# anonymous-author-918/deq-mpc-corl

Hardware: AMD Instinct MI355X
Metric: QP solves/sec at (B,T=20,nx=13,nu=4) (higher is better)
Workload: dtype f32

## Files before the change

deq-mpc-corl_amd/_lib.py:

```python
from __future__ import annotations

import ctypes as C
import os

_HERE = os.path.dirname(os.path.abspath(__file__))
LIB_PATH = os.environ.get("MI_ALQP_LIB") or os.path.join(_HERE, "csrc", "libmi_alqp.so")

ABI_VERSION = 10


class AlqpDims(C.Structure):
    _fields_ = [("B", C.c_int), ("T", C.c_int), ("nx", C.c_int), ("nu", C.c_int)]


class AlqpParams(C.Structure):
    _fields_ = [("al_iter", C.c_int), ("max_newton", C.c_int), ("n_ls", C.c_int),
                ("flags", C.c_int), ("rho_scale", C.c_double), ("variant", C.c_int),
                ("skip_flag", C.c_void_p), ("exit_tol", C.c_double), ("newton_counts", C.c_void_p),
                ("exit_scratch", C.c_void_p), ("quad_stagger", C.c_int)]


class AlqpTrace(C.Structure):
    _fields_ = [("g", C.c_void_p), ("d", C.c_void_p), ("phi", C.c_void_p),
                ("phi_prev", C.c_void_p), ("k", C.c_void_p), ("accept", C.c_void_p)]


class AlqpObstacles(C.Structure):
    _fields_ = [("pos", C.c_void_p), ("radius", C.c_double), ("nobs", C.c_int), ("state_estimator", C.c_int)]


class AlqpIpmParams(C.Structure):
    _fields_ = [("flags", C.c_int), ("max_iter", C.c_int), ("iter0", C.c_int), ("kkt_eps", C.c_double),
                ("variant", C.c_int)]


class AlqpRigidParams(C.Structure):
    _fields_ = [("mass", C.c_double), ("J", C.c_double * 9), ("Jinv", C.c_double * 9), ("g", C.c_double * 3),
                ("motor_dist", C.c_double), ("kf", C.c_double), ("bf", C.c_double), ("km", C.c_double),
                ("act_scale", C.c_double), ("u_hover", C.c_double), ("pend_L", C.c_double), ("ss", C.c_double * 12),
                ("bf_force", C.c_double)]


IPM_VARIANTS = {"auto": 0, "generic_lds": 1, "generic_ws": 2, "resident": 3}


ALQP_IPM_INIT, ALQP_IPM_RESID, ALQP_IPM_STEP, ALQP_IPM_LOOP, ALQP_IPM_FINAL = 1, 2, 4, 8, 16
ALQP_INIT_MERIT = 1
ALQP_DUAL_UPDATE = 2
ALQP_SAVE_FACTOR = 4
ALQP_WS_PRIMED = 8
ALQP_EXIT_IN_KERNEL = 16
ALQP_E_COOP = -4
# ... 19 lines not shown
                                   C.c_long, C.c_long, _P, _P, _P, _P, _P]),
    "alqp_merit": (C.c_int, [C.POINTER(AlqpDims), C.c_int, _P, _P, _P, _P, _P, _P, _P, _P, _P,
                             C.c_long, C.c_long, _P, _P, _P]),
    "alqp_linesearch_pick": (C.c_int, [C.POINTER(AlqpDims), C.c_int, _P, _P, _P, _P, _P, _P, _P]),
    "alqp_dual_update": (C.c_int, [C.POINTER(AlqpDims), _P, _P, _P, _P, _P, C.c_long, C.c_long, _P, _P,
                                   C.c_double, _P]),
    "alqp_backward": (C.c_int, [C.POINTER(AlqpDims), _P, _P, _P, _P, _P, _P, _P, _P]),
    "alqp_backward_ws": (C.c_int, [C.POINTER(AlqpDims), _P, C.c_size_t, _P, _P, _P, _P, _P, _P, _P]),
    "alqp_newton_step_obs": (C.c_int, [C.POINTER(AlqpDims), _P, _P, _P, _P, _P, _P, _P, _P, _P, _P,
                                       C.c_long, C.c_long, C.POINTER(AlqpObstacles), _P, _P, _P, _P, _P]),
    "alqp_merit_obs": (C.c_int, [C.POINTER(AlqpDims), C.c_int, _P, _P, _P, _P, _P, _P, _P, _P, _P,
                                 C.c_long, C.c_long, C.POINTER(AlqpObstacles), _P, _P, _P]),
    "alqp_dual_update_obs": (C.c_int, [C.POINTER(AlqpDims), _P, _P, _P, _P, _P, C.c_long, C.c_long,
                                       C.POINTER(AlqpObstacles), _P, _P, C.c_double, _P]),
    "alqp_newton_step_ws": (C.c_int, [C.POINTER(AlqpDims), _P, _P, _P, _P, _P, _P, _P, _P, _P, _P,
                                      C.c_long, C.c_long, _P, C.c_size_t, _P, _P, _P, _P]),
    "alqp_newton_step_ws_obs": (C.c_int, [C.POINTER(AlqpDims), _P, _P, _P, _P, _P, _P, _P, _P, _P, _P,
                                          C.c_long, C.c_long, C.POINTER(AlqpObstacles), _P, C.c_size_t, _P, _P, _P, _P]),
    "alqp_merit_pick": (C.c_int, [C.POINTER(AlqpDims), C.c_int, _P, _P, _P, _P, _P, _P, _P, _P, _P,
                                  C.c_long, C.c_long, C.POINTER(AlqpObstacles), _P, _P, _P, _P, _P, _P, _P]),
    "alqp_ipm_solve": (C.c_int, [C.POINTER(AlqpDims), C.POINTER(AlqpIpmParams), _P, _P, _P, _P, _P, _P, _P,
                                 C.c_long, C.c_long, C.c_long, C.c_long, C.c_long, C.c_long, _P, C.c_size_t, _P,
                                 _P, _P, _P, _P, _P, _P, _P, _P, _P, _P]),
    "alqp_ipm_backward": (C.c_int, [C.POINTER(AlqpDims), _P, _P, C.c_long, C.c_long, C.c_long, C.c_long, _P, _P, _P,
                                    _P, C.c_size_t, _P, _P, _P, _P, C.c_int, _P]),
}
_PLAIN = {
    "alqp_abi_version": (C.c_int, []),
    "alqp_supported": (C.c_int, [C.POINTER(AlqpDims), C.c_int]),
    "alqp_supported_variant": (C.c_int, [C.POINTER(AlqpDims), C.c_int, C.c_int]),
    "alqp_lds_bytes": (C.c_size_t, [C.POINTER(AlqpDims), C.c_int]),
    "alqp_qps_per_wave": (C.c_int, [C.POINTER(AlqpDims), C.c_int]),
    "alqp_workspace_bytes": (C.c_size_t, [C.POINTER(AlqpDims), C.c_int]),
    "alqp_exit_test": (C.c_int, [C.c_void_p, C.c_void_p, C.c_int, C.c_double, C.c_void_p]),
    "alqp_workspace_bytes_nonlin": (C.c_size_t, [C.POINTER(AlqpDims), C.c_int]),
    "alqp_ipm_workspace_bytes": (C.c_size_t, [C.POINTER(AlqpDims), C.c_int]),
}

EXPORTED_SYMBOLS = sorted([f"{n}_{s}" for n in _SIGS for s in ("f32", "f64")] + list(_PLAIN))

_lib = None


def load():
    global _lib
    if _lib is not None:
        return _lib
    if not os.path.exists(LIB_PATH):
        raise RuntimeError(
            f"mi_alqp: HIP extension not built ({LIB_PATH} missing). Run "
            "`python -c 'import __graft_entry__ as g; g.build()'` - there is no CPU fallback.")
    lib = C.CDLL(LIB_PATH)
    for name, (res, args) in _SIGS.items():
        for sfx in ("f32", "f64"):
            fn = getattr(lib, f"{name}_{sfx}")
            fn.restype = res
            fn.argtypes = args
    for name, (res, args) in _PLAIN.items():
        fn = getattr(lib, name)
        fn.restype = res
        fn.argtypes = args
    if lib.alqp_abi_version() != ABI_VERSION:
        raise RuntimeError("mi_alqp: libmi_alqp.so ABI version mismatch - rebuild the extension")
    _lib = lib
    return lib

# ... 5 lines not shown
```

deq-mpc-corl_amd/backend.py:

```python
from __future__ import annotations

import ctypes as C

import os

import torch

from . import _lib


def _dt(t):
    if t.dtype == torch.float32:
        return "f32"
    if t.dtype == torch.float64:
        return "f64"
    raise TypeError(f"mi_alqp: unsupported dtype {t.dtype}")


def _ptr(t, name, dtype=None, allow_none=False):
    if t is None:
        if allow_none:
            return None
        raise ValueError(f"mi_alqp: {name} is required")
    if not t.is_cuda:
# ... 15 lines not shown


class HipBackend:

    name = "hip"
    supports_exit_in_kernel = True
    default_variant = "auto"
    QUAD_MIN_BATCH = 4096

    def __init__(self):
        self.lib = _lib.load()
        self._ws = {}
        if os.environ.get("ALQP_QUAD_STAGGER") is not None:
            self.set_quad_stagger(int(os.environ["ALQP_QUAD_STAGGER"]))

    quad_stagger = -1

    def set_quad_stagger(self, mode):
        prev, self.quad_stagger = self.quad_stagger, (-1 if int(mode) < 0 else int(mode))
        return prev

    def workspace_bytes(self, B, T, nx, nu, dtype):
        d = _lib.AlqpDims(B, T, nx, nu)
        return int(self.lib.alqp_workspace_bytes(C.byref(d), int(dtype == torch.float64)))

    def _workspace(self, dims, like):
        need = self.workspace_bytes(*dims, like.dtype)
        key = (like.device, like.dtype)
        ws = self._ws.get(key)
        if ws is None or ws.numel() * ws.element_size() < need:
            ws = torch.empty(need // like.element_size() + 16, dtype=like.dtype, device=like.device)
            self._ws[key] = ws
        return ws, need

    def supported(self, B, T, nx, nu, dtype):
        d = _lib.AlqpDims(B, T, nx, nu)
        return bool(self.lib.alqp_supported(C.byref(d), int(dtype == torch.float64)))

    def lds_bytes(self, B, T, nx, nu, dtype):
        d = _lib.AlqpDims(B, T, nx, nu)
        return int(self.lib.alqp_lds_bytes(C.byref(d), int(dtype == torch.float64)))

    def qps_per_wave(self, B, T, nx, nu, dtype):
        d = _lib.AlqpDims(B, T, nx, nu)
        return int(self.lib.alqp_qps_per_wave(C.byref(d), int(dtype == torch.float64)))

    def solve_lin(self, dims, Qd, q, F, c, x0, ulo, uhi, sb_u, st_u, z, lam, rho, phi,
                  rnorm2=None, info=None, status=None, factor=None, al_iter=2, max_newton=4,
                  n_ls=20, flags=_lib.ALQP_INIT_MERIT | _lib.ALQP_DUAL_UPDATE, rho_scale=10.0,
                  trace=None, variant=None, workspace=None, skip=None, newton_counts=None, exit_tol=1e-3):
        B, T, nx, nu = dims
        dt = z.dtype
        sfx = _dt(z)
        d = _lib.AlqpDims(B, T, nx, nu)
        if variant is None:
            variant = self.default_variant
        vnum = {"auto": 0, "team": 1, "quad": 2}[variant]
        if vnum == 0:
            if self.QUAD_MIN_BATCH != 4096:
                qmin = self.QUAD_MIN_BATCH
            elif 2 * (nx + nu) + nx + 1 > 32:
                qmin = 4097
            else:
                qmin = 4608 if dt == torch.float64 else 4096
            vnum = 1 if ((flags & _lib.ALQP_SAVE_FACTOR) or B < qmin) else 2
            if vnum == 1 and not (flags & _lib.ALQP_SAVE_FACTOR) and not self.lib.alqp_supported_variant(C.byref(d), int(dt == torch.float64), 1):
                vnum = 2
        ws, ws_bytes = (None, 0)
        if vnum == 2:
            if workspace is not None:
                ws, ws_bytes = workspace, self.workspace_bytes(*dims, z.dtype)
                if ws.numel() * ws.element_size() < ws_bytes:
                    raise ValueError("mi_alqp: workspace too small")
            else:
                ws, ws_bytes = self._workspace(dims, z)
        self.last_variant = "quad" if vnum == 2 else "team"
        skp = _ptr(skip, "skip", torch.float64, True)
        p = _lib.AlqpParams(al_iter, max_newton, n_ls, flags | _DEBUG_FLAGS, rho_scale, vnum, skp.value if skp is not None else None)
        p.quad_stagger = {-1: 0, 0: -1}.get(self.quad_stagger, self.quad_stagger)
        if newton_counts is not None:
            self._exit_in_kernel(p, B, z.device, newton_counts, exit_tol)
        tr = None
        if trace is not None:
            tr = _lib.AlqpTrace(*[
                (trace[k].data_ptr() if trace.get(k) is not None else None)
                for k in ("g", "d", "phi", "phi_prev", "k", "accept")])
        fn = getattr(self.lib, "alqp_solve_lin_" + sfx)
        rc = fn(C.byref(d), C.byref(p), _ptr(Qd, "Qd", dt), _ptr(q, "q", dt), _ptr(F, "F", dt),
                _ptr(c, "c", dt), _ptr(x0, "x0", dt), _ptr(ulo, "u_lower", dt), _ptr(uhi, "u_upper", dt),
                sb_u, st_u, _ptr(z, "z", dt), _ptr(lam, "lam", dt), _ptr(rho, "rho", dt),
                _ptr(phi, "phi", dt), _ptr(rnorm2, "rnorm2", dt, True),
                _ptr(info, "info", torch.int32, True), _ptr(status, "status", torch.uint8, True),
                _ptr(factor, "factor", dt, True), C.byref(tr) if tr is not None else None,
                _ptr(ws, "workspace", dt, True), ws_bytes, _stream())
        if rc == _lib.ALQP_E_COOP and newton_counts is not None:
            return False
        _lib.check(rc, "alqp_solve_lin_" + sfx)
        return True

    def _exit_in_kernel(self, p, B, device, newton_counts, exit_tol):
        key = ("exit", device)
        scr = self._ws.get(key)
        if scr is None or scr.numel() < 2 * B + 2:
            scr = torch.zeros(2 * B + 2, dtype=torch.float64, device=device)
            self._ws[key] = scr
        scr.zero_()
        p.flags |= _lib.ALQP_EXIT_IN_KERNEL
        p.exit_tol = float(exit_tol)
        p.newton_counts = _ptr(newton_counts, "newton_counts", torch.int32).value
        p.exit_scratch = scr.data_ptr()

    def solve_nonlin(self, dims, dyn_id, dyn_h, Qd, q, x0, ulo, uhi, sb_u, st_u, z, lam, rho, phi, rnorm2=None,
# ... 337 lines not shown
```

deq-mpc-corl_amd/csrc/alqp_kernels.hip:

```cpp
#include <hip/hip_runtime.h>

#include "alqp_team.hpp"
#include "alqp_quad.hpp"
#include "mi_alqp.h"
#include "alqp_dims.hpp"

#ifndef ALQP_PART
#define ALQP_PART 0
#endif
#define ALQP_BUILD_MAIN (ALQP_PART == 0 || ALQP_PART == 1)
#define ALQP_BUILD_QUAD (ALQP_PART == 0 || ALQP_PART == 2 || ALQP_PART == 3)
#define ALQP_QUAD_F32 (ALQP_PART == 0 || ALQP_PART == 2)
#define ALQP_QUAD_F64 (ALQP_PART == 0 || ALQP_PART == 3)

#include <hip/hip_cooperative_groups.h>

namespace alqp {

template <typename real>
struct SolveArgs {
    int B, T;
    int al_iter, max_newton, n_ls, flags;
    real rho_scale;
    const real *Qd, *q, *F, *c, *x0, *ulo, *uhi;
    long sb_u, st_u;
    real *z, *lam, *rho, *phi, *rnorm2;
    int *info;
    unsigned char *status;
    real *factor;
    const double *skip;
    real dyn_h;
    int stagger;
    double exit_tol;
    int *newton_counts;
    double *exit_scratch;
};

__device__ inline double grid_sum_ordered(double block_val, double *scratch, int &phase) {
    double *p = scratch + 1 + (size_t)(phase & 1) * gridDim.x;
    unsigned *cnt = reinterpret_cast<unsigned *>(scratch);
    double *timed_out = scratch + 1 + 2 * (size_t)gridDim.x;
    if (threadIdx.x == 0) {
        __hip_atomic_store(p + blockIdx.x, block_val, __ATOMIC_RELAXED, __HIP_MEMORY_SCOPE_AGENT);
        __hip_atomic_fetch_add(cnt, 1u, __ATOMIC_RELEASE, __HIP_MEMORY_SCOPE_AGENT);
        const unsigned target = (unsigned)(phase + 1) * gridDim.x;
        if (__hip_atomic_load(timed_out, __ATOMIC_RELAXED, __HIP_MEMORY_SCOPE_AGENT) == 0.0) {
            const unsigned long long t0 = __builtin_amdgcn_s_memrealtime();
            bool late = false;
            while (__hip_atomic_load(cnt, __ATOMIC_RELAXED, __HIP_MEMORY_SCOPE_AGENT) < target) {
                __builtin_amdgcn_s_sleep(2);
                if (__builtin_amdgcn_s_memrealtime() - t0 > 100000000ull ||
                    __hip_atomic_load(timed_out, __ATOMIC_RELAXED, __HIP_MEMORY_SCOPE_AGENT) != 0.0) { late = true; break; }
            }
            if (late) __hip_atomic_store(timed_out, 1.0, __ATOMIC_RELAXED, __HIP_MEMORY_SCOPE_AGENT);
            else (void)__hip_atomic_load(cnt, __ATOMIC_ACQUIRE, __HIP_MEMORY_SCOPE_AGENT);
        }
    }
    __builtin_amdgcn_s_barrier();
    if (__hip_atomic_load(timed_out, __ATOMIC_RELAXED, __HIP_MEMORY_SCOPE_AGENT) != 0.0) {
        ++phase;
        return __builtin_nan("");
    }
    double s = 0;
    for (unsigned i = threadIdx.x; i < gridDim.x; i += 64) s += __hip_atomic_load(p + i, __ATOMIC_RELAXED, __HIP_MEMORY_SCOPE_AGENT);
#pragma unroll
    for (int off = 32; off; off >>= 1) s += __shfl_xor(s, off, 64);
    ++phase;
    return s;
// ... 190 lines not shown
    }

    const real rn2 = tm.rplus2();
    int bad = 0;
    for (int e = li; e < T * N; e += G) {
        real v = tm.zs[e];
        bad |= !(v - v == real(0));
    }
    bad = team_or<G>(bad);
#ifdef ALQP_PHASE_TIMING
    tm.stamp(7);
    if (lane == 0)
        for (int i = 0; i < 8; ++i) atomicAdd(&g_team_cycles[i], tm.tacc[i]);
#endif
    if (active) {
        for (int e = li; e < T * N; e += G) gz[e] = tm.zs[e];
        if ((a.flags & ALQP_SAVE_FACTOR) && a.factor) {
            real *gf = a.factor + (size_t)b * T * C::XT;
            for (int e = li; e < T * C::XT; e += G) gf[e] = tm.Xp[e];
        }
        if (li == 0) {
            a.rho[b] = tm.rho;
            a.phi[b] = phi_prev;
            if (a.rnorm2) a.rnorm2[b] = rn2;
            if (a.info && tm.info && a.info[b] == 0) a.info[b] = tm.info;
            if (a.status) a.status[b] = bad ? 0 : 1;
        }
    }
}

#endif

#if ALQP_BUILD_QUAD
#ifndef ALQP_FUSE_LS
#define ALQP_FUSE_LS 1
#endif
#ifdef ALQP_PHASE_TIMING
__device__ unsigned long long g_phase_cycles[10];
#define QSTAMP(b) qd.stamp(b)
#else
#define QSTAMP(b)
#endif
template <typename real, int NX, int NU, bool TRACE, class Dyn = NoDyn>
__global__ __launch_bounds__(64) __attribute__((amdgpu_waves_per_eu(1, 1))) void k_solve_lin_quad(SolveArgs<real> a, TraceArgs<real> tr, real *ws) {
    using C = QCfg<real, NX, NU>;
    constexpr bool NL = Dyn::ID != 0;
#ifndef ALQP_FUSE_LS_F64
#define ALQP_FUSE_LS_F64 1
#endif
    constexpr bool FUSE_LS = ALQP_FUSE_LS && (sizeof(real) == 4 || ALQP_FUSE_LS_F64) && !NL;
    constexpr int N = C::N;
    if (a.skip && *a.skip != 0.0) return;
    const int lane = threadIdx.x, qi = lane >> 2;
    const int b_raw = blockIdx.x * 16 + qi;
    const bool active = b_raw < a.B;
    {
        int stag = a.stagger;
        const int mode = (a.flags >> 20) & 0xf;
        if ((a.flags >> 24) & 0xff) stag = (a.flags >> 24) & 0xff;
        if (stag > 0) {
            const unsigned hw = __builtin_amdgcn_s_getreg(4 | (0 << 6) | (31 << 11));
            int simd = (hw >> 4) & 3;
            if (mode == 1) simd = simd * 16 + ((hw >> 8) & 0xf);
            if (mode == 2) simd &= 1;
            if (mode == 3) simd = blockIdx.x & 1;
            if (mode == 4) simd = (simd & 1) ^ (blockIdx.x & 1);
            if (mode == 5) simd = (hw >> 8) & 3;
            for (int i = 0; i < simd * stag; ++i) __builtin_amdgcn_s_sleep(16);
        }
    }
#ifdef ALQP_ALIAS_ALL
    const int b = (active ? b_raw : a.B - 1) % ALQP_ALIAS_ALL;
#else
    const int b = active ? b_raw : a.B - 1;
#endif
    const int T = a.T, M = C::M(T);

    Quad<real, NX, NU> qd;
    __shared__ real w_lds[QCfg<real, NX, NU>::WLDS_WORDS];
    qd.wl = w_lds + threadIdx.x;
    qd.q = lane & 3;
    qd.T = T;
    qd.active = active;
    qd.gQd = a.Qd + (size_t)b * T * N;
    qd.gq = a.q + (size_t)b * T * N;
    qd.gF = a.F + (size_t)b * (T - 1) * NX * N;
    qd.gc = a.c + (size_t)b * (T - 1) * NX;
    qd.gx0 = a.x0 + (size_t)b * NX;
    qd.gulo = a.ulo + (size_t)b * a.sb_u;
    qd.guhi = a.uhi + (size_t)b * a.sb_u;
    qd.st_u = a.st_u;
    qd.gz = a.z + (size_t)b * T * N;
    qd.glam = a.lam + (size_t)b * M;
    qd.rec = ws + C::rec_base(b, T);
    qd.gFw = const_cast<real *>(qd.gF);
    qd.dyn_h = a.dyn_h;
    qd.rho = a.rho[b];
    qd.info = 0;
    real phi_prev = a.phi[b];
#ifdef ALQP_PHASE_TIMING
    for (int i = 0; i < 10; ++i) qd.tacc[i] = 0;
#endif
    QSTAMP(-1);
    if (!(a.flags & ALQP_WS_PRIMED)) {
        if constexpr (NL) qd.stage_in(false, false);
        else qd.stage_in(a.max_newton == 0 || a.al_iter == 0 || (a.flags & ALQP_EXIT_IN_KERNEL) ||
                         (!C::PHI0_FWD && (a.flags & ALQP_INIT_MERIT)));
    }
    const bool ref_exit = (a.flags & ALQP_EXIT_IN_KERNEL) != 0;
    int gphase = 0;

    int step_id = 0;
    bool pend = false;
    real alpha_pend = 0;
    int bad = 0;
    real rn2 = 0, phi_next = 0;
    for (int it = 0; it < a.al_iter; ++it) {
        bool phi_from_forward = false;
        if (a.flags & ALQP_INIT_MERIT) {
            if (it > 0) {
                phi_prev = phi_next;
            } else if (C::PHI0_FWD && a.max_newton > 0 && !ref_exit) {
                phi_from_forward = true;
            } else {
                if constexpr (NL) qd.template linearize<Dyn>(real(0), false);
                real p1[1];
                qd.template merit_candidates<1>(p1, true);
                phi_prev = p1[0];
            }
        }
        pend = false;
        double nrm_old = 0;
        int n_done = 0;
        if (ref_exit) {
            int bad0 = 0;
            const real r0 = it == 0 ? qd.rplus2(bad0) : rn2;
            nrm_old = sqrt(grid_sum_ordered(wave_sum_leaders(exit_term(r0, qor(qd.info)), active && qd.q == 0), a.exit_scratch, gphase));
        }
        for (int st = 0; st < a.max_newton; ++st, ++step_id) {
            real *tg = nullptr;
            if constexpr (TRACE) tg = (tr.g && active) ? tr.g + ((size_t)step_id * a.B + b) * T * N : nullptr;
            QSTAMP(9);
            if constexpr (NL) {
                qd.template linearize<Dyn>(alpha_pend, pend);
                pend = false;
            }
            qd.forward(tg, alpha_pend, pend, (phi_from_forward && st == 0) ? &phi_prev : nullptr);
            real ph[20];
            qd.template backward<FUSE_LS>(ph);
            QSTAMP(-1);
            if constexpr (TRACE) {
                if (tr.d && active) {
                    real *td = tr.d + ((size_t)step_id * a.B + b) * T * N;
                    for (int t = 0; t < T; ++t)
                        for (int j = qd.q; j < N; j += 4) td[t * N + j] = qd.recp(t)[C::wn(C::oY, j)];
                }
            }
            if constexpr (NL) qd.template merit_nonlin<Dyn>(ph);
            else if constexpr (!FUSE_LS) qd.template merit_candidates<20>(ph, false);
            QSTAMP(6);
            int kbest = 0;
            real best = ph[0];
#pragma unroll
            for (int k = 1; k < 20; ++k) {
                if (k < a.n_ls && !(best != best) && (ph[k] != ph[k] || ph[k] < best)) {
                    best = ph[k];
                    kbest = k;
                }
            }
            const bool acc = best < phi_prev;
            if constexpr (TRACE) {
                if (active && qd.q == 0) {
                    if (tr.phi)
#pragma unroll
                        for (int k = 0; k < 20; ++k)
                            if (k < a.n_ls) tr.phi[((size_t)step_id * a.n_ls + k) * a.B + b] = ph[k];
                    if (tr.phi_prev) tr.phi_prev[(size_t)step_id * a.B + b] = phi_prev;
                    if (tr.k) tr.k[(size_t)step_id * a.B + b] = kbest;
                    if (tr.accept) tr.accept[(size_t)step_id * a.B + b] = acc ? 1 : 0;
                }
// ... 577 lines not shown
#undef X
    return ALQP_E_UNSUPPORTED;
}

#if ALQP_QUAD_F32
template int dispatch_step_quad<float>(int, int, const StepArgs<float> &, float *, hipStream_t);
#endif
#if ALQP_QUAD_F64
template int dispatch_step_quad<double>(int, int, const StepArgs<double> &, double *, hipStream_t);
#endif

#if ALQP_QUAD_F32
template int dispatch_solve_nonlin<float>(int, int, int, const SolveArgs<float> &, float *, hipStream_t);
template int dispatch_solve_quad<float>(int, int, const SolveArgs<float> &, const TraceArgs<float> *, float *, hipStream_t);
template int dispatch_backward_quad<float>(int, int, const BwdArgs<float> &, float *, hipStream_t);
#endif
#if ALQP_QUAD_F64
template int dispatch_solve_nonlin<double>(int, int, int, const SolveArgs<double> &, double *, hipStream_t);
template int dispatch_solve_quad<double>(int, int, const SolveArgs<double> &, const TraceArgs<double> *, double *, hipStream_t);
template int dispatch_backward_quad<double>(int, int, const BwdArgs<double> &, double *, hipStream_t);
#endif

#endif

template <typename real>
size_t quad_ws_bytes(int nx, int nu, int B, int T) {
#define X(NX, NU) \
    if (nx == NX && nu == NU) return QCfg<real, NX, NU>::ws_covers(B, T) ? QCfg<real, NX, NU>::ws_words(B, T) * sizeof(real) : 0;
    ALQP_FOR_EACH_DIMS(X)
#undef X
    return 0;
}

#if ALQP_BUILD_MAIN
template <typename real>
int dispatch_step(int nx, int nu, const StepArgs<real> &a, hipStream_t stream) {
#define X(NX, NU) \
    if (nx == NX && nu == NU) return launch_team_kernel<real, NX, NU>(k_newton_step<real, NX, NU>, a.B, a.T, stream, a);
    ALQP_FOR_EACH_DIMS(X)
#undef X
    return ALQP_E_UNSUPPORTED;
}

template <typename real>
int dispatch_backward(int nx, int nu, const BwdArgs<real> &a, hipStream_t stream) {
#define X(NX, NU) \
    if (nx == NX && nu == NU) return launch_team_kernel<real, NX, NU>(k_backward<real, NX, NU>, a.B, a.T, stream, a);
    ALQP_FOR_EACH_DIMS(X)
#undef X
    return ALQP_E_UNSUPPORTED;
}

template <typename real>
size_t lds_query(int nx, int nu, int T) {
#define X(NX, NU) \
    if (nx == NX && nu == NU) return lds_bytes_for<real, NX, NU>(T);
    ALQP_FOR_EACH_DIMS(X)
#undef X
    return 0;
}

static int qpw_query(int nx, int nu) {
#define X(NX, NU) \
    if (nx == NX && nu == NU) return Cfg<float, NX, NU>::QPW;
    ALQP_FOR_EACH_DIMS(X)
#undef X
// ... 39 lines not shown
    a.B = dims->B; a.T = dims->T;
    a.al_iter = prm->al_iter; a.max_newton = prm->max_newton; a.n_ls = prm->n_ls; a.flags = prm->flags;
    a.rho_scale = (real)prm->rho_scale;
    a.Qd = (const real *)Qd; a.q = (const real *)q; a.F = (const real *)F; a.c = (const real *)c;
    a.x0 = (const real *)x0; a.ulo = (const real *)u_lo; a.uhi = (const real *)u_hi;
    a.sb_u = sb_u; a.st_u = st_u;
    a.z = (real *)z; a.lam = (real *)lam; a.rho = (real *)rho; a.phi = (real *)phi;
    a.rnorm2 = (real *)rnorm2; a.info = info; a.status = status; a.factor = (real *)factor_out;
    a.skip = prm->skip_flag;
    a.stagger = quad_stagger(prm->quad_stagger, dims->B, dims->T, dims->nx, dims->nu, prm->al_iter * prm->max_newton, sizeof(real) == 8);
    if (prm->flags & ALQP_EXIT_IN_KERNEL) {
        if (!prm->exit_scratch || trace || prm->skip_flag) return ALQP_E_BADARG;
        a.exit_tol = prm->exit_tol; a.newton_counts = prm->newton_counts; a.exit_scratch = prm->exit_scratch;
    }
    TraceArgs<real> tr = {};
    if (trace) {
        tr.g = (real *)trace->g; tr.d = (real *)trace->d; tr.phi = (real *)trace->phi;
        tr.phi_prev = (real *)trace->phi_prev; tr.k = trace->k; tr.accept = trace->accept;
    }
    const size_t need = quad_ws_bytes<real>(dims->nx, dims->nu, dims->B, dims->T);
    int variant = prm->variant;
    if (variant == 0) {
        const size_t team_lds = lds_query<real>(dims->nx, dims->nu, dims->T);
        const bool team_fits = team_lds > 0 && team_lds <= kMaxLds;
        const bool quad_ok = need > 0 && workspace && ws_bytes >= need && !(prm->flags & ALQP_SAVE_FACTOR);
        const bool wave_team = 2 * (dims->nx + dims->nu) + dims->nx + 1 > 32;
        const int qmin = wave_team ? 4097 : (sizeof(real) == 8 ? 4608 : 4096);
        variant = (quad_ok && (dims->B >= qmin || !team_fits)) ? 2 : 1;
    }
    if (variant == 2) {
        if (prm->flags & ALQP_SAVE_FACTOR) return ALQP_E_UNSUPPORTED;
        if (need == 0) return ALQP_E_UNSUPPORTED;
        if (!workspace || ws_bytes < need) return ALQP_E_BADARG;
        return dispatch_solve_quad<real>(dims->nx, dims->nu, a, trace ? &tr : nullptr, (real *)workspace,
                                         (hipStream_t)stream);
    }
    if (variant != 1) return ALQP_E_BADARG;
    return dispatch_solve<real>(dims->nx, dims->nu, a, trace ? &tr : nullptr, (hipStream_t)stream);
}

template <typename real>
size_t nonlin_ws_bytes(int nx, int nu, int B, int T) {
    const size_t rec = quad_ws_bytes<real>(nx, nu, B, T);
    if (rec == 0) return 0;
    return rec + (size_t)B * (T - 1) * nx * (nx + nu) * sizeof(real);
}

template <typename real>
int solve_nonlin_impl(const AlqpDims *dims, const AlqpParams *prm, int dyn_id, double dyn_h, const void *Qd, const void *q,
                      const void *x0, const void *u_lo, const void *u_hi, long sb_u, long st_u, void *z, void *lam,
                      void *rho, void *phi, void *rnorm2, int *info, unsigned char *status, void *workspace,
                      size_t ws_bytes, void *stream) {
    if (!dims_ok(dims) || !prm || !Qd || !q || !x0 || !u_lo || !u_hi || !z || !lam || !rho || !phi || !workspace)
        return ALQP_E_BADARG;
    if (prm->n_ls != 20 || prm->al_iter < 0 || prm->max_newton < 0) return ALQP_E_BADARG;
    if (prm->flags & (ALQP_SAVE_FACTOR | ALQP_WS_PRIMED)) return ALQP_E_UNSUPPORTED;
    const size_t need = nonlin_ws_bytes<real>(dims->nx, dims->nu, dims->B, dims->T);
    if (need == 0) return ALQP_E_UNSUPPORTED;
    if (ws_bytes < need) return ALQP_E_BADARG;
    SolveArgs<real> a = {};
    a.B = dims->B; a.T = dims->T;
    a.al_iter = prm->al_iter; a.max_newton = prm->max_newton; a.n_ls = prm->n_ls; a.flags = prm->flags;
    a.rho_scale = (real)prm->rho_scale;
    a.Qd = (const real *)Qd; a.q = (const real *)q; a.c = nullptr; a.x0 = (const real *)x0;
    a.F = (const real *)((const char *)workspace + quad_ws_bytes<real>(dims->nx, dims->nu, dims->B, dims->T));
    a.ulo = (const real *)u_lo; a.uhi = (const real *)u_hi; a.sb_u = sb_u; a.st_u = st_u;
// ... 329 lines not shown
    }
}

template <typename real>
int dyn_cartpole2l_impl(long K, const void *x, const void *tau, double h, const void *hpt, void *xn, void *J, void *stream) {
    if (K < 0 || !x || !tau || (!xn && !J)) return ALQP_E_BADARG;
    if (K == 0) return 0;
    hipLaunchKernelGGL(k_dyn_cartpole2l<real>, dim3((unsigned)((K + 127) / 128)), dim3(128), 0, (hipStream_t)stream, K,
                       (const real *)x, (const real *)tau, (real)h, (const real *)hpt, (real *)xn, (real *)J);
    return hipGetLastError() == hipSuccess ? 0 : ALQP_E_LAUNCH;
}

__global__ void k_exit_test(const double *sumsq, double *ctl, int mode, double tol) {
    if (threadIdx.x != 0 || blockIdx.x != 0) return;
    const double nw = sqrt(sumsq[0]);
    if (mode == 0) {
        ctl[0] = 0.0;
        ctl[1] = 0.0;
        ctl[2] = nw;
    } else if (ctl[0] == 0.0) {
        ctl[1] += 1.0;
        const double old = ctl[2];
        if (nw < tol || fabs(old - nw) / nw < tol) ctl[0] = 1.0;
        else ctl[2] = nw;
    }
}
#endif

}

#if ALQP_BUILD_MAIN
extern "C" {

int alqp_abi_version(void) { return 10; }

int alqp_dyn_pendulum1l_f32(long K, const void *x, const void *u, double h, const void *h_pt, void *xnext, void *F, void *stream) {
    return alqp::dyn_pendulum1l_impl<float>(K, x, u, h, h_pt, xnext, F, stream);
}
int alqp_dyn_pendulum1l_f64(long K, const void *x, const void *u, double h, const void *h_pt, void *xnext, void *F, void *stream) {
    return alqp::dyn_pendulum1l_impl<double>(K, x, u, h, h_pt, xnext, F, stream);
}

int alqp_dyn_cartpole1l_f32(long K, const void *x, const void *tau, double h, const void *h_pt, void *xnext, void *J, void *stream) {
    return alqp::dyn_cartpole1l_impl<float>(K, x, tau, h, h_pt, xnext, J, stream);
}
int alqp_dyn_cartpole1l_f64(long K, const void *x, const void *tau, double h, const void *h_pt, void *xnext, void *J, void *stream) {
    return alqp::dyn_cartpole1l_impl<double>(K, x, tau, h, h_pt, xnext, J, stream);
}
int alqp_dyn_cartpole1l_v2_f32(long K, const void *x, const void *tau, double h, const void *h_pt, void *xnext, void *J, void *stream) {
    return alqp::dyn_cartpole1l_impl<float>(K, x, tau, h, h_pt, xnext, J, stream, 2);
}
int alqp_dyn_cartpole1l_v2_f64(long K, const void *x, const void *tau, double h, const void *h_pt, void *xnext, void *J, void *stream) {
    return alqp::dyn_cartpole1l_impl<double>(K, x, tau, h, h_pt, xnext, J, stream, 2);
}

int alqp_dyn_cartpole2l_f32(long K, const void *x, const void *tau, double h, const void *h_pt, void *xnext, void *J, void *stream) {
    return alqp::dyn_cartpole2l_impl<float>(K, x, tau, h, h_pt, xnext, J, stream);
}
int alqp_dyn_cartpole2l_f64(long K, const void *x, const void *tau, double h, const void *h_pt, void *xnext, void *J, void *stream) {
    return alqp::dyn_cartpole2l_impl<double>(K, x, tau, h, h_pt, xnext, J, stream);
}

size_t alqp_workspace_bytes_nonlin(const AlqpDims *dims, int is_f64) {
    if (!alqp::dims_ok(dims)) return 0;
    return is_f64 ? alqp::nonlin_ws_bytes<double>(dims->nx, dims->nu, dims->B, dims->T)
                  : alqp::nonlin_ws_bytes<float>(dims->nx, dims->nu, dims->B, dims->T);
}
int alqp_solve_nonlin_f32(const AlqpDims *dims, const AlqpParams *prm, int dyn_id, double dyn_h, const void *Qd,
                          const void *q, const void *x0, const void *u_lo, const void *u_hi, long sb_u, long st_u, void *z,
                          void *lam, void *rho, void *phi, void *rnorm2, int *info, unsigned char *status, void *workspace,
                          size_t ws_bytes, void *stream) {
    return alqp::solve_nonlin_impl<float>(dims, prm, dyn_id, dyn_h, Qd, q, x0, u_lo, u_hi, sb_u, st_u, z, lam, rho, phi,
                                          rnorm2, info, status, workspace, ws_bytes, stream);
}
int alqp_solve_nonlin_f64(const AlqpDims *dims, const AlqpParams *prm, int dyn_id, double dyn_h, const void *Qd,
                          const void *q, const void *x0, const void *u_lo, const void *u_hi, long sb_u, long st_u, void *z,
                          void *lam, void *rho, void *phi, void *rnorm2, int *info, unsigned char *status, void *workspace,
                          size_t ws_bytes, void *stream) {
    return alqp::solve_nonlin_impl<double>(dims, prm, dyn_id, dyn_h, Qd, q, x0, u_lo, u_hi, sb_u, st_u, z, lam, rho, phi,
                                           rnorm2, info, status, workspace, ws_bytes, stream);
}

int alqp_exit_test(const double *sumsq, double *ctl, int mode, double tol, void *stream) {
    if (!sumsq || !ctl || (mode != 0 && mode != 1)) return ALQP_E_BADARG;
    hipLaunchKernelGGL(alqp::k_exit_test, dim3(1), dim3(64), 0, (hipStream_t)stream, sumsq, ctl, mode, tol);
    return hipGetLastError() == hipSuccess ? 0 : ALQP_E_LAUNCH;
}

size_t alqp_workspace_bytes(const AlqpDims *dims, int is_f64) {
    if (!alqp::dims_ok(dims)) return 0;
    return is_f64 ? alqp::quad_ws_bytes<double>(dims->nx, dims->nu, dims->B, dims->T)
                  : alqp::quad_ws_bytes<float>(dims->nx, dims->nu, dims->B, dims->T);
}

size_t alqp_lds_bytes(const AlqpDims *dims, int is_f64) {
    if (!alqp::dims_ok(dims)) return 0;
    size_t v = is_f64 ? alqp::lds_query<double>(dims->nx, dims->nu, dims->T)
                      : alqp::lds_query<float>(dims->nx, dims->nu, dims->T);
    return v;
}

int alqp_supported(const AlqpDims *dims, int is_f64) {
    return alqp_workspace_bytes(dims, is_f64) > 0;
}

int alqp_supported_variant(const AlqpDims *dims, int is_f64, int variant) {
    if (variant == 2) return alqp_workspace_bytes(dims, is_f64) > 0;
    if (variant == 1) {
        size_t v = alqp_lds_bytes(dims, is_f64);
        return v > 0 && v <= alqp::kMaxLds;
    }
    return 0;
}

int alqp_qps_per_wave(const AlqpDims *dims, int is_f64) {
    (void)is_f64;
    if (!alqp::dims_ok(dims)) return 0;
    return alqp::qpw_query(dims->nx, dims->nu);
}

#define ALQP_DEFINE(SFX, REAL)                                                                        \
    int alqp_solve_lin_##SFX(const AlqpDims *dims, const AlqpParams *prm, const void *Qd,             \
                             const void *q, const void *F, const void *c, const void *x0,             \
                             const void *u_lo, const void *u_hi, long sb_u, long st_u, void *z,       \
                             void *lam, void *rho, void *phi, void *rnorm2, int *info,                \
// ... 141 lines not shown
```

deq-mpc-corl_amd/csrc/alqp_quad.hpp:

```cpp
#pragma once
#include <hip/hip_runtime.h>

#include <type_traits>

#include "alqp_team.hpp"
#include "alqp_dyn.hpp"

namespace alqp {

template <int Q>
__device__ inline float qb(float v) {
    return __builtin_bit_cast(float, __builtin_amdgcn_mov_dpp(__builtin_bit_cast(int, v), Q * 0x55, 0xF, 0xF, true));
}
template <int Q>
__device__ inline double qb(double v) {
    long long b = __builtin_bit_cast(long long, v);
    int lo = __builtin_amdgcn_mov_dpp((int)(b & 0xffffffffll), Q * 0x55, 0xF, 0xF, true);
    int hi = __builtin_amdgcn_mov_dpp((int)(b >> 32), Q * 0x55, 0xF, 0xF, true);
    return __builtin_bit_cast(double, ((long long)hi << 32) | (unsigned int)lo);
}
template <typename real>
__device__ inline real qbv(real v, int src) {
    switch (src & 3) {
        case 0: return qb<0>(v);
// ... 169 lines not shown
        for (int k = 2; k < i; ++k) o += 16 * (fslots(k) / 4);
        return o;
    }
    static constexpr FldT<head_at(0), tail_at(0)> oY{};
    static constexpr FldT<head_at(1), tail_at(1)> oZ{};
    static constexpr FldT<head_at(2), tail_at(2)> oR{};
    static constexpr FldT<head_at(3), tail_at(3)> oS{};
    static constexpr FldT<head_at(4), tail_at(4)> oLE{};
    static_assert(NU <= 4, "the u-slot layout holds one control per lane");
    static constexpr FldT<head_at(5), tail_at(5)> oUS{};
    static constexpr FldT<head_at(6), tail_at(6)> oQ{};
    static constexpr FldT<head_at(7), tail_at(7)> oq{};
    static constexpr FldT<head_at(8), tail_at(8)> oC{};
    static constexpr int RECW = (head_at(NF) + 31) & ~31;
    static_assert(IL == 1 || RECW % 16 == 0, "whole groups per record");
    template <int S>
    __host__ __device__ static constexpr int lp(int m, int q) {
        return m < 4 * (S / 4) ? 16 * (m / 4) + 4 * q + m % 4 : 16 * (S / 4) + q * (S % 4) + m - 4 * (S / 4);
    }
    template <int S>
    __host__ __device__ static constexpr int fw(Fld f, int p) {
        return p < 16 * (S / 4) ? w(f.h + p) : w(f.t + 4 * ((p - 16 * (S / 4)) / (S % 4)) + (p - 16 * (S / 4)) % (S % 4));
    }
    __host__ __device__ static constexpr int pn(int k) { return lp<SY>(k >> 2, k & 3); }
    __host__ __device__ static constexpr int px(int r) { return lp<SW>(r >> 2, r & 3); }
    __host__ __device__ static constexpr int wn(Fld f, int k) { return fw<SY>(f, pn(k)); }
    __host__ __device__ static constexpr int M(int T) { return T * NX + 2 * T * NU; }
    static constexpr int RSTR = RECW * IL;
    __host__ __device__ static constexpr size_t rec_base(int b, int T) { return (size_t)(b / IL) * T * RSTR + (size_t)(b % IL) * 16; }
    __host__ __device__ static constexpr size_t ws_words(int B, int T) { return (size_t)((B + IL - 1) / IL) * T * RSTR; }
    __host__ static bool ws_covers(int B, int T) {
        return rec_base(B - 1, T) + (size_t)(T - 1) * RSTR + w(RECW - 1) + 1 <= ws_words(B, T);
    }
};

template <typename real, int NX, int NU>
struct Quad {
    using C = QCfg<real, NX, NU>;
    static constexpr int N = C::N, SH = C::SH, SW = C::SW, SY = C::SY, HT = C::HT, ST = C::ST, RECW = C::RECW;

    int q, T;
    bool active;
    const real *gQd, *gq, *gF, *gc, *gx0, *gulo, *guhi;
    long st_u;
    real *gz, *glam, *rec;
    real rho;
    int info;
    real *wl;
    using WT = WPanel<real, SW, N, C::W_LDS>;
    __device__ __forceinline__ WT wpanel() const {
        if constexpr (C::W_LDS) return WT{wl};
        else return WT{};
    }
    real *gFw;
    real dyn_h;
    const real *gobs;
    int nobs;
    real obs_r2;
    bool no_init;

    __device__ __forceinline__ real uhi(int t, int j) const { return guhi[t * st_u + j]; }
    __device__ __forceinline__ real ulo(int t, int j) const { return gulo[t * st_u + j]; }
    __device__ __forceinline__ real *recp(int t) const { return rec + (size_t)t * C::RSTR; }
#ifdef ALQP_PHASE_TIMING
    unsigned long long tacc[10], tlast;
    __device__ __forceinline__ void stamp(int bucket) {
        unsigned long long now;
        __builtin_amdgcn_sched_barrier(0);
        asm volatile("s_waitcnt vmcnt(0)\n\ts_memtime %0\n\ts_waitcnt lgkmcnt(0)" : "=s"(now)::"memory");
        __builtin_amdgcn_sched_barrier(0);
        if (bucket >= 0) tacc[bucket] += now - tlast;
        tlast = now;
    }
#define ALQP_STAMP(b) stamp(b)
#else
#define ALQP_STAMP(b)
#endif

    template <int S, int L>
    __device__ __forceinline__ void ld_slots(FRef<real> f, real (&v)[L]) const {
        static_assert(L <= S, "slots of the field");
#pragma unroll
        for (int c = 0; 4 * c < L && c < S / 4; ++c) {
            const real *p = f.p + C::w(f.f.h + 16 * c) + 4 * q;
            if (4 * c + 3 < L) gld4(p, v[4 * c], v[4 * c + 1], v[4 * c + 2], v[4 * c + 3]);
            else
#pragma unroll
// ... 74 lines not shown
            const int k = 4 * m + q;
            const real x = src[(4 * m + 3 < LEN || k < LEN) ? k : LEN - 1];
            v[m] = (4 * m + 3 < LEN || k < LEN) ? x : real(0);
        }
    }
    template <int LEN, int SL>
    __device__ __forceinline__ void st_own_ext(real *dst, const real (&v)[SL]) const {
#pragma unroll
        for (int m = 0; m < SL; ++m)
            if (4 * m + 3 < LEN || 4 * m + q < LEN) dst[4 * m + q] = v[m];
    }

    __device__ __forceinline__ int own_ju() const { return (q - NX) & 3; }
    __device__ __forceinline__ void ld_own_us(const real *rp, real &lu, real &ll, real &bu, real &bl) const {
        gld4(rp + C::w(C::oUS.h) + 4 * q, lu, ll, bu, bl);
    }
    __device__ __forceinline__ void st_own_us(real *rp, real lu, real ll, real bu, real bl) const {
        gst4(rp + C::w(C::oUS.h) + 4 * q, lu, ll, bu, bl);
    }
    __device__ __forceinline__ void ld_rep_us(const real *rp, real (&lu)[NU], real (&ll)[NU], real (&bu)[NU], real (&bl)[NU]) const {
        real w[16];
        ld_field<4>(rp + C::oUS, w);
#pragma unroll
        for (int ju = 0; ju < NU; ++ju) {
            const int ql = (NX + ju) & 3;
            lu[ju] = w[4 * ql];
            ll[ju] = w[4 * ql + 1];
            bu[ju] = w[4 * ql + 2];
            bl[ju] = w[4 * ql + 3];
        }
    }

    __device__ __forceinline__ void load_F_rows(int t, WT &W) const {
        const real *Fg = gF + (size_t)t * NX * N;
#pragma unroll
        for (int s = 0; s < SW; ++s) {
            const int r = 4 * s + q;
            const int rc = (4 * s + 3 < NX) ? r : (r < NX ? r : NX - 1);
            gload<N>(Fg + rc * N, W[s]);
            if (4 * s + 3 >= NX) {
                const real m = r < NX ? real(1) : real(0);
#pragma unroll
                for (int k = 0; k < N; ++k) W[s][k] *= m;
            }
        }
    }
    template <int LEN>
    __device__ __forceinline__ void copy_slice(const real *src, real *dst) const {
#pragma unroll
        for (int c = 0; 16 * c < LEN; ++c) {
            const int w0 = 16 * c + 4 * q;
            if (16 * c + 15 < LEN || w0 + 3 < LEN) {
                real a, b, cc, d;
                gld4(src + w0, a, b, cc, d);
                gst4(dst + w0, a, b, cc, d);
            } else {
#pragma unroll
                for (int w = 0; w < 4; ++w)
                    if (w0 + w < LEN) dst[w0 + w] = src[w0 + w];
            }
        }
    }
    __device__ __forceinline__ void stage_in(bool with_residual, bool have_c = true) {
#pragma unroll 2
        for (int t = 0; t < T; ++t) {
            const bool dyn = t < T - 1;
            real *rp = recp(t);
            if (active) {
                real vn[SY], vx[SW];
                ld_own_ext<N>(gz + t * N, vn);
                st_own_n(rp + C::oZ, vn);
                ld_own_ext<N>(gQd + t * N, vn);
                st_own_n(rp + C::oQ, vn);
                ld_own_ext<N>(gq + t * N, vn);
                st_own_n(rp + C::oq, vn);
                ld_own_ext<NX>(glam + t * NX, vx);
                st_own_x(rp + C::oLE, vx);
                {
// ... 269 lines not shown
                    real dt[SY], dn[SW];
                    ld_own_n(rp + C::oY, dt);
                    ld_ownx_of_n(rn + C::oY, dn);
#pragma unroll
                    for (int m = 0; m < SY; ++m) zs[m] = fma_(alpha, dt[m], zs[m]);
#pragma unroll
                    for (int s = 0; s < SW; ++s) zn[s] = fma_(alpha, dn[s], zn[s]);
                }
                ALQP_STAMP(0);
#pragma unroll
                for (int k = 0; k < N; ++k) zt[k] = qbv(zs[k >> 2], k);
                real rro[SW];
                if (!dyn) {
#pragma unroll
                    for (int s = 0; s < SW; ++s)
#pragma unroll
                        for (int k = 0; k < N; ++k) W[s][k] = 0;
                }
#pragma unroll
                for (int s = 0; s < SW; ++s) {
                    const int r = 4 * s + q;
                    real xn = cs[s];
                    if constexpr (!EXT) {
#pragma unroll
                        for (int k = 0; k < N; ++k) xn = fma_(W[s][k], zt[k], xn);
                    }
                    const real rr = zn[s] - xn;
                    const bool ok = dyn && r < NX;
                    v[s] = ok ? fma_(rho, rr, lm[s]) : real(0);
                    rro[s] = ok ? rr : real(0);
                    if constexpr (C::PHI0_FWD) mdist += ok ? fma_(fma_(real(0.5) * rho, rr, lm[s]), rr, real(0)) : real(0);
                }
                if (!ALQP_EXP_NORS && !EXT && dyn && active) st_own_x(rp + C::oR, rro);
                constexpr int MU0 = NX / 4;
                real zu = 0;
#pragma unroll
                for (int m = MU0; m < SY; ++m) zu = (4 * m + q >= NX && 4 * m + q < N) ? zs[m] : zu;
                const real vu = zu - bu, vl = bl - zu;
                const real au = vu >= 0 ? real(1) : real(0), al = vl >= 0 ? real(1) : real(0);
                const real cu = fmax_(vu, real(0)), cl = fmax_(vl, real(0));
                const real gu = fma_(rho, cu, lu) - fma_(rho, cl, ll);
                const real du = rho * (au + al);
                if constexpr (C::PHI0_FWD)
                    mdist += own_ju() < NU ? fma_(lu, vu, ll * vl) + real(0.5) * rho * fma_(cu, cu, cl * cl) : real(0);
                real go[SY];
#pragma unroll
                for (int m = 0; m < SY; ++m) {
                    const int j = 4 * m + q;
                    const bool isx = (4 * m + 3 < NX) ? true : (4 * m >= NX ? false : j < NX);
                    const bool isu = (4 * m + 3 < NX) ? false : (j >= NX && j < N);
                    real g = fma_(Qo[m], zs[m], qo[m]);
                    real d = Qo[m];
                    if constexpr (C::PHI0_FWD) mdist = fma_(fma_(real(0.5) * Qo[m], zs[m], qo[m]), zs[m], mdist);
                    g += isx ? vpo[m < SW ? m : 0] : (isu ? gu : real(0));
                    bool pinned = isx;
                    if constexpr (EXT) {
                        pinned = isx && !(no_init && t == 0);
                        if (no_init && isu) g = 0;
                    }
                    d += pinned ? rho : (isu ? du : real(0));
                    dio[m] = d;
                    go[m] = g;
                }
                if constexpr (EXT && NX >= 3) {
                    if (nobs > 0) {
                        const real *lk = glam + T * NX + t * (2 * NU + nobs) + 2 * NU;
// ... 656 lines not shown
```

include/mi_alqp.h:

```cpp
#ifndef MI_ALQP_H
#define MI_ALQP_H

#include <stddef.h>

#ifdef __cplusplus
extern "C" {
#endif

typedef struct AlqpDims {
    int B;
    int T;
    int nx;
    int nu;
} AlqpDims;

typedef struct AlqpObstacles {
    const void *pos;
    double radius;
    int nobs;
    int state_estimator;
} AlqpObstacles;

#define ALQP_INIT_MERIT   1
#define ALQP_DUAL_UPDATE  2
#define ALQP_SAVE_FACTOR  4
#define ALQP_WS_PRIMED    8

#define ALQP_EXIT_IN_KERNEL 16

typedef struct AlqpParams {
    int al_iter;
    int max_newton;
    int n_ls;
    int flags;
    double rho_scale;
    int variant;
    const double *skip_flag;
    double exit_tol;
    int *newton_counts;
    double *exit_scratch;
    int quad_stagger;
} AlqpParams;

typedef struct AlqpTrace {
    void *g;
    void *d;
    void *phi;
    void *phi_prev;
    int *k;
    int *accept;
} AlqpTrace;

#define ALQP_E_BADARG     (-1)
#define ALQP_E_UNSUPPORTED (-2)
#define ALQP_E_LAUNCH     (-3)
#define ALQP_E_COOP       (-4)

int alqp_supported(const AlqpDims *dims, int is_f64);
int alqp_supported_variant(const AlqpDims *dims, int is_f64, int variant);
size_t alqp_lds_bytes(const AlqpDims *dims, int is_f64);
int alqp_qps_per_wave(const AlqpDims *dims, int is_f64);
size_t alqp_workspace_bytes(const AlqpDims *dims, int is_f64);

int alqp_solve_lin_f32(const AlqpDims *dims, const AlqpParams *prm, const void *Qd, const void *q,
                       const void *F, const void *c, const void *x0, const void *u_lo,
                       const void *u_hi, long sb_u, long st_u, void *z, void *lam, void *rho,
                       void *phi, void *rnorm2, int *info, unsigned char *status,
                       void *factor_out, const AlqpTrace *trace, void *workspace, size_t ws_bytes,
                       void *stream);
int alqp_solve_lin_f64(const AlqpDims *dims, const AlqpParams *prm, const void *Qd, const void *q,
                       const void *F, const void *c, const void *x0, const void *u_lo,
                       const void *u_hi, long sb_u, long st_u, void *z, void *lam, void *rho,
                       void *phi, void *rnorm2, int *info, unsigned char *status,
                       void *factor_out, const AlqpTrace *trace, void *workspace, size_t ws_bytes,
                       void *stream);

int alqp_newton_step_f32(const AlqpDims *dims, const void *z, const void *xnext, const void *F,
                         const void *x0, const void *lam, const void *rho, const void *Qd,
                         const void *q, const void *u_lo, const void *u_hi, long sb_u, long st_u,
                         void *d_out, void *g_out, void *factor_out, int *info, void *stream);
int alqp_newton_step_f64(const AlqpDims *dims, const void *z, const void *xnext, const void *F,
                         const void *x0, const void *lam, const void *rho, const void *Qd,
                         const void *q, const void *u_lo, const void *u_hi, long sb_u, long st_u,
                         void *d_out, void *g_out, void *factor_out, int *info, void *stream);

int alqp_newton_step_ws_f32(const AlqpDims *dims, const void *z, const void *xnext, const void *F,
                            const void *x0, const void *lam, const void *rho, const void *Qd, const void *q,
                            const void *u_lo, const void *u_hi, long sb_u, long st_u, void *workspace,
                            size_t ws_bytes, void *d_out, void *g_out, int *info, void *stream);
int alqp_newton_step_ws_f64(const AlqpDims *dims, const void *z, const void *xnext, const void *F,
                            const void *x0, const void *lam, const void *rho, const void *Qd, const void *q,
                            const void *u_lo, const void *u_hi, long sb_u, long st_u, void *workspace,
                            size_t ws_bytes, void *d_out, void *g_out, int *info, void *stream);

int alqp_merit_f32(const AlqpDims *dims, int K, const void *zc, const void *xnext, const void *x0,
// ... 157 lines not shown
```

Baseline: 5.993 million.

## Cache dynamics Jacobian in a coalesced lane-packed image for quad solver

After: 5.315 million (median of 2 runs). -11.3%, worse.

```diff
diff --git a/deq-mpc-corl_amd/_lib.py b/deq-mpc-corl_amd/_lib.py
--- a/deq-mpc-corl_amd/_lib.py
+++ b/deq-mpc-corl_amd/_lib.py
@@ -6,7 +6,7 @@
 _HERE = os.path.dirname(os.path.abspath(__file__))
 LIB_PATH = os.environ.get("MI_ALQP_LIB") or os.path.join(_HERE, "csrc", "libmi_alqp.so")
 
-ABI_VERSION = 10
+ABI_VERSION = 11
 
 
 class AlqpDims(C.Structure):
@@ -17,7 +17,8 @@
     _fields_ = [("al_iter", C.c_int), ("max_newton", C.c_int), ("n_ls", C.c_int),
                 ("flags", C.c_int), ("rho_scale", C.c_double), ("variant", C.c_int),
                 ("skip_flag", C.c_void_p), ("exit_tol", C.c_double), ("newton_counts", C.c_void_p),
-                ("exit_scratch", C.c_void_p), ("quad_stagger", C.c_int)]
+                ("exit_scratch", C.c_void_p), ("quad_stagger", C.c_int), ("f_image", C.c_void_p),
+                ("f_image_bytes", C.c_size_t)]
 
 
 class AlqpTrace(C.Structure):
@@ -103,6 +104,7 @@
     "alqp_lds_bytes": (C.c_size_t, [C.POINTER(AlqpDims), C.c_int]),
     "alqp_qps_per_wave": (C.c_int, [C.POINTER(AlqpDims), C.c_int]),
     "alqp_workspace_bytes": (C.c_size_t, [C.POINTER(AlqpDims), C.c_int]),
+    "alqp_fimage_bytes": (C.c_size_t, [C.POINTER(AlqpDims), C.c_int]),
     "alqp_exit_test": (C.c_int, [C.c_void_p, C.c_void_p, C.c_int, C.c_double, C.c_void_p]),
     "alqp_workspace_bytes_nonlin": (C.c_size_t, [C.POINTER(AlqpDims), C.c_int]),
     "alqp_ipm_workspace_bytes": (C.c_size_t, [C.POINTER(AlqpDims), C.c_int]),
diff --git a/deq-mpc-corl_amd/backend.py b/deq-mpc-corl_amd/backend.py
--- a/deq-mpc-corl_amd/backend.py
+++ b/deq-mpc-corl_amd/backend.py
@@ -71,6 +71,18 @@
             ws = torch.empty(need // like.element_size() + 16, dtype=like.dtype, device=like.device)
             self._ws[key] = ws
         return ws, need
+
+    def _fimage(self, dims, like):
+        d = _lib.AlqpDims(*dims)
+        need = int(self.lib.alqp_fimage_bytes(C.byref(d), int(like.dtype == torch.float64)))
+        if need == 0:
+            return None, 0
+        key = (like.device, like.dtype, "fimage")
+        img = self._ws.get(key)
+        if img is None or img.numel() * img.element_size() < need:
+            img = torch.empty(need // like.element_size(), dtype=like.dtype, device=like.device)
+            self._ws[key] = img
+        return img, need
 
     def supported(self, B, T, nx, nu, dtype):
         d = _lib.AlqpDims(B, T, nx, nu)
@@ -117,6 +129,9 @@
         skp = _ptr(skip, "skip", torch.float64, True)
         p = _lib.AlqpParams(al_iter, max_newton, n_ls, flags | _DEBUG_FLAGS, rho_scale, vnum, skp.value if skp is not None else None)
         p.quad_stagger = {-1: 0, 0: -1}.get(self.quad_stagger, self.quad_stagger)
+        if vnum == 2:
+            img, p.f_image_bytes = self._fimage(dims, z)
+            p.f_image = img.data_ptr() if img is not None else None
         if newton_counts is not None:
             self._exit_in_kernel(p, B, z.device, newton_counts, exit_tol)
         tr = None
diff --git a/deq-mpc-corl_amd/csrc/alqp_kernels.hip b/deq-mpc-corl_amd/csrc/alqp_kernels.hip
--- a/deq-mpc-corl_amd/csrc/alqp_kernels.hip
+++ b/deq-mpc-corl_amd/csrc/alqp_kernels.hip
@@ -34,6 +34,7 @@
     double exit_tol;
     int *newton_counts;
     double *exit_scratch;
+    real *fimg;
 };
 
 __device__ inline double grid_sum_ordered(double block_val, double *scratch, int &phase) {
@@ -290,6 +291,9 @@
 #endif
 
 #if ALQP_BUILD_QUAD
+#ifndef ALQP_EXP_FLINES
+#define ALQP_EXP_FLINES 0
+#endif
 #ifndef ALQP_FUSE_LS
 #define ALQP_FUSE_LS 1
 #endif
@@ -355,6 +359,17 @@
     qd.dyn_h = a.dyn_h;
     qd.rho = a.rho[b];
     qd.info = 0;
+    bool fimg = false;
+    if constexpr (C::FIMG && !NL) {
+#if ALQP_EXP_FLINES
+        qd.fimg = ws + C::fimg_base(b, T);
+        fimg = true;
+#else
+        fimg = a.fimg != nullptr;
+        qd.fimg = fimg ? a.fimg + C::fimg_base(b, T) : nullptr;
+        qd.fimg_wr = fimg;
+#endif
+    }
     real phi_prev = a.phi[b];
 #ifdef ALQP_PHASE_TIMING
     for (int i = 0; i < 10; ++i) qd.tacc[i] = 0;
@@ -404,6 +419,8 @@
                 pend = false;
             }
             qd.forward(tg, alpha_pend, pend, (phi_from_forward && st == 0) ? &phi_prev : nullptr);
+            qd.fimg_wr = false;
+            qd.fimg_rd = fimg;
             real ph[20];
             qd.template backward<FUSE_LS>(ph);
             QSTAMP(-1);
@@ -1047,6 +1064,15 @@
     return 0;
 }
 
+template <typename real>
+size_t quad_fimage_bytes(int nx, int nu, int B, int T) {
+#define X(NX, NU) \
+    if (nx == NX && nu == NU) return QCfg<real, NX, NU>::fimg_words(B, T) * sizeof(real);
+    ALQP_FOR_EACH_DIMS(X)
+#undef X
+    return 0;
+}
+
 #if ALQP_BUILD_MAIN
 template <typename real>
 int dispatch_step(int nx, int nu, const StepArgs<real> &a, hipStream_t stream) {
@@ -1152,6 +1178,11 @@
         if (prm->flags & ALQP_SAVE_FACTOR) return ALQP_E_UNSUPPORTED;
         if (need == 0) return ALQP_E_UNSUPPORTED;
         if (!workspace || ws_bytes < need) return ALQP_E_BADARG;
+        const size_t fneed = quad_fimage_bytes<real>(dims->nx, dims->nu, dims->B, dims->T);
+        if (prm->f_image && fneed > 0) {
+            if (prm->f_image_bytes < fneed || (reinterpret_cast<uintptr_t>(prm->f_image) & 127)) return ALQP_E_BADARG;
+            a.fimg = (real *)prm->f_image;
+        }
         return dispatch_solve_quad<real>(dims->nx, dims->nu, a, trace ? &tr : nullptr, (real *)workspace,
                                          (hipStream_t)stream);
     }
@@ -1547,7 +1578,7 @@
 #if ALQP_BUILD_MAIN
 extern "C" {
 
-int alqp_abi_version(void) { return 10; }
+int alqp_abi_version(void) { return 11; }
 
 int alqp_dyn_pendulum1l_f32(long K, const void *x, const void *u, double h, const void *h_pt, void *xnext, void *F, void *stream) {
     return alqp::dyn_pendulum1l_impl<float>(K, x, u, h, h_pt, xnext, F, stream);
@@ -1606,6 +1637,12 @@
     if (!alqp::dims_ok(dims)) return 0;
     return is_f64 ? alqp::quad_ws_bytes<double>(dims->nx, dims->nu, dims->B, dims->T)
                   : alqp::quad_ws_bytes<float>(dims->nx, dims->nu, dims->B, dims->T);
+}
+
+size_t alqp_fimage_bytes(const AlqpDims *dims, int is_f64) {
+    if (!alqp::dims_ok(dims)) return 0;
+    return is_f64 ? alqp::quad_fimage_bytes<double>(dims->nx, dims->nu, dims->B, dims->T)
+                  : alqp::quad_fimage_bytes<float>(dims->nx, dims->nu, dims->B, dims->T);
 }
 
 size_t alqp_lds_bytes(const AlqpDims *dims, int is_f64) {
diff --git a/deq-mpc-corl_amd/csrc/alqp_quad.hpp b/deq-mpc-corl_amd/csrc/alqp_quad.hpp
--- a/deq-mpc-corl_amd/csrc/alqp_quad.hpp
+++ b/deq-mpc-corl_amd/csrc/alqp_quad.hpp
@@ -225,6 +225,20 @@
     __host__ static bool ws_covers(int B, int T) {
         return rec_base(B - 1, T) + (size_t)(T - 1) * RSTR + w(RECW - 1) + 1 <= ws_words(B, T);
     }
+    static constexpr int FSF = NX / 4, FNC = N / 4;
+    static constexpr bool FIMG = sizeof(real) == 4 && NX % 4 == 1 && N % 4 == 1 && FNC <= 4 && SW <= 4;
+    static constexpr int FG_ROW = FNC * FSF, FG_COL = FG_ROW + 1, FG = FG_COL + 1;
+    static constexpr int FSTR = 2 * 16 * FG;
+    __host__ __device__ static constexpr int fgw(int g) { return 32 * g; }
+    __host__ __device__ static constexpr size_t fimg_base(int b, int T) { return (size_t)(b / 2) * (T - 1) * FSTR + (size_t)(b % 2) * 16; }
+    __host__ __device__ static constexpr size_t fimg_words(int B, int T) {
+        return FIMG && T > 1 ? (size_t)((B + 1) / 2) * (T - 1) * FSTR : 0;
+    }
+    __host__ __device__ static constexpr int fimg_el(int g, int q, int i) {
+        if (g < FG_ROW) return (4 * (g / FNC) + q) * N + 4 * (g % FNC) + i;
+        if (g == FG_ROW) return q < FNC ? (NX - 1) * N + 4 * q + i : -1;
+        return i < SW && 4 * i + q < NX ? (4 * i + q) * N + N - 1 : -1;
+    }
 };
 
 template <typename real, int NX, int NU>
@@ -246,6 +260,8 @@
         else return WT{};
     }
     real *gFw;
+    real *fimg = nullptr;
+    bool fimg_wr = false, fimg_rd = false;
     real dyn_h;
     const real *gobs;
     int nobs;
@@ -386,6 +402,12 @@
     }
 
     __device__ __forceinline__ void load_F_rows(int t, WT &W) const {
+        if constexpr (C::FIMG) {
+            if (fimg_rd) {
+                load_F_image(t, W);
+                return;
+            }
+        }
         const real *Fg = gF + (size_t)t * NX * N;
 #pragma unroll
         for (int s = 0; s < SW; ++s) {
@@ -398,6 +420,43 @@
                 for (int k = 0; k < N; ++k) W[s][k] *= m;
             }
         }
+    }
+    __device__ __forceinline__ void load_F_image(int t, WT &W) const {
+        const real *p = fimg + (size_t)t * C::FSTR + 4 * q;
+#pragma unroll
+        for (int s = 0; s < C::FSF; ++s)
+#pragma unroll
+            for (int c = 0; c < C::FNC; ++c)
+                gld4(p + C::fgw(C::FNC * s + c), W[s][4 * c], W[s][4 * c + 1], W[s][4 * c + 2], W[s][4 * c + 3]);
+        real lr[4], lc[4];
+        gld4(p + C::fgw(C::FG_ROW), lr[0], lr[1], lr[2], lr[3]);
+        gld4(p + C::fgw(C::FG_COL), lc[0], lc[1], lc[2], lc[3]);
+        const real m = q == 0 ? real(1) : real(0);
+#pragma unroll
+        for (int c = 0; c < C::FNC; ++c)
+#pragma unroll
+            for (int i = 0; i < 4; ++i) W[C::FSF][4 * c + i] = qbv(lr[i], c) * m;
+#pragma unroll
+        for (int s = 0; s < SW; ++s) W[s][N - 1] = s == C::FSF ? lc[s] * m : lc[s];
+    }
+    __device__ __forceinline__ void store_F_image(int t, const WT &W) const {
+        real *p = fimg + (size_t)t * C::FSTR + 4 * q;
+#pragma unroll
+        for (int s = 0; s < C::FSF; ++s)
+#pragma unroll
+            for (int c = 0; c < C::FNC; ++c)
+                gst4(p + C::fgw(C::FNC * s + c), W[s][4 * c], W[s][4 * c + 1], W[s][4 * c + 2], W[s][4 * c + 3]);
+        real lr[4], lc[4];
+#pragma unroll
+        for (int i = 0; i < 4; ++i) {
+            real x[4];
+#pragma unroll
+            for (int c = 0; c < 4; ++c) x[c] = c < C::FNC ? qb<0>(W[C::FSF][c < C::FNC ? 4 * c + i : 0]) : real(0);
+            lr[i] = sel4(x[0], x[1], x[2], x[3], q);
+            lc[i] = i < SW ? W[i < SW ? i : 0][N - 1] : real(0);
+        }
+        gst4(p + C::fgw(C::FG_ROW), lr[0], lr[1], lr[2], lr[3]);
+        gst4(p + C::fgw(C::FG_COL), lc[0], lc[1], lc[2], lc[3]);
     }
     template <int LEN>
     __device__ __forceinline__ void copy_slice(const real *src, real *dst) const {
@@ -733,6 +792,9 @@
                     if constexpr (C::PHI0_FWD) mdist += ok ? fma_(fma_(real(0.5) * rho, rr, lm[s]), rr, real(0)) : real(0);
                 }
                 if (!ALQP_EXP_NORS && !EXT && dyn && active) st_own_x(rp + C::oR, rro);
+                if constexpr (C::FIMG && !EXT) {
+                    if (fimg_wr && dyn && active) store_F_image(t, W);
+                }
                 constexpr int MU0 = NX / 4;
                 real zu = 0;
 #pragma unroll
diff --git a/include/mi_alqp.h b/include/mi_alqp.h
--- a/include/mi_alqp.h
+++ b/include/mi_alqp.h
@@ -40,6 +40,8 @@
     int *newton_counts;
     double *exit_scratch;
     int quad_stagger;
+    void *f_image;
+    size_t f_image_bytes;
 } AlqpParams;
 
 typedef struct AlqpTrace {
@@ -61,6 +63,7 @@
 size_t alqp_lds_bytes(const AlqpDims *dims, int is_f64);
 int alqp_qps_per_wave(const AlqpDims *dims, int is_f64);
 size_t alqp_workspace_bytes(const AlqpDims *dims, int is_f64);
+size_t alqp_fimage_bytes(const AlqpDims *dims, int is_f64);
 
 int alqp_solve_lin_f32(const AlqpDims *dims, const AlqpParams *prm, const void *Qd, const void *q,
                        const void *F, const void *c, const void *x0, const void *u_lo,
```
